# MP-Gadget/MP-Gadget

Measured on AMD Instinct MI355X. Metric: particle-updates/sec (gravity force step: PM + tree build + short-range walk), higher is better.
Workload: dtype f64; 1 GPU; 256^3 DM-only TreePM force step, Nmesh=512, s_zel ICs, all particles active, relative opening criterion (ErrTolForceAcc 0.002), TreeRcut 6, Asmth 1.5; particles=16777216, nmesh=512, parallelism=1 GPU

## Files before the change

mp-gadget_amd/csrc/grav_walk_split.hip:

```cpp
#include "grav_walk.h"
#include <cstdlib>
#include <cstring>
#include <cstdio>
#include <type_traits>

namespace mpg {

namespace {

constexpr int EVAL_BLOCKS = 4;
constexpr int LIST_BLOCKS = 6;

__device__ __forceinline__ double rsqrt_nr(double x)
{
    const double y = __builtin_amdgcn_rsq(x);
    const double e = fma(-(x * y), y, 1.0);
    return fma(y * e, fma(e, 0.375, 0.5), y);
}

template <unsigned long long BITS>
__device__ __forceinline__ double scalar_literal()
{
    unsigned lo, hi;
    asm volatile("s_mov_b32 %0, %2\n\ts_mov_b32 %1, %3" : "=s"(lo), "=s"(hi) : "i"((unsigned)(BITS & 0xffffffffull)), "i"((unsigned)(BITS >> 32)));
    return __hiloint2double((int)hi, (int)lo);
}
#define MPG_K(x) scalar_literal<__builtin_bit_cast(unsigned long long, (double)(x))>()

__device__ __forceinline__ double rcp_nr(double x)
{
    double y = __builtin_amdgcn_rcp(x);
    y = fma(fma(-x, y, 1.0), y, y);
    return fma(fma(-x, y, 1.0), y, y);
}

__device__ __forceinline__ void softened_pair(const double r0, const double r2, const double rinv, const double m, const double h, const double hinv,
                                              const double h3inv, double &fac, double &facpot)
{
    const double r = fma(fma(-r0, r0, r2), 0.5 * rinv, r0);
    const double q = r * hinv;
    const double u = fma(fma(-q, h, r), hinv, q);
    double wpk;
    if(u < 0.5) {
        fac = m * h3inv * (MPG_K(10.666666666667) + u * u * (MPG_K(32.0) * u - MPG_K(38.4)));
        wpk = MPG_K(-2.8) + u * u * (MPG_K(5.333333333333) + u * u * (MPG_K(6.4) * u - MPG_K(9.6)));
    }
    else {
        const double iu = rcp_nr(u);
        fac = m * h3inv * (MPG_K(21.333333333333) - MPG_K(48.0) * u + MPG_K(38.4) * u * u - MPG_K(10.666666666667) * u * u * u -
                           MPG_K(0.066666666667) * (iu * iu * iu));
        wpk = MPG_K(-3.2) + MPG_K(0.066666666667) * iu +
              u * u * (MPG_K(10.666666666667) + u * (MPG_K(-16.0) + u * (MPG_K(9.6) - MPG_K(2.133333333333) * u)));
    }
    facpot = m * hinv * wpk;
}

struct PairTmp {
    double dx, dy, dz, r2, rinv, r, fac, facpot, m;
};

__device__ __forceinline__ void pair_pre(const Src4 s, const double dx, const double dy, const double dz, PairTmp &t)
{
    t.dx = dx;
    t.dy = dy;
    t.dz = dz;
    t.m = s.m;
    t.r2 = dx * dx + dy * dy + dz * dz;
    t.rinv = rsqrt_nr(t.r2);
    t.r = t.r2 * t.rinv;
    const double mr = s.m * t.rinv;
    t.fac = mr * t.rinv * t.rinv;
    t.facpot = -mr;
}

__device__ __forceinline__ void pair_soft(const GravParams &gp, PairTmp &t)
{
    if(t.r2 == 0.0) {
        t.r = 0.0;
        t.fac = t.m * gp.h3inv * 10.666666666667;
        t.facpot = t.m * gp.hinv * -2.8;
    }
    else {
        if(!(t.rinv < 1e150)) {
            t.r = 0.0;
            t.rinv = 0.0;
        }
        softened_pair(t.r, t.r2, t.rinv, t.m, gp.h, gp.hinv, gp.h3inv, t.fac, t.facpot);
    }
}

template <bool POT>
__device__ __forceinline__ void pair_post(const PairTmp &t, const GravParams &gp, const double *__restrict__ wtab, double &ax, double &ay, double &az,
                                          double &pot)
{
    const double ti = t.r * gp.inv_cell_dx;
    const int ix = min((int)ti, NTAB - 1);
    const double w1 = __builtin_amdgcn_fract(ti);
    const double *__restrict__ row = wtab + ix * 2;
    const double2 f = *(const double2 *)row;
    double2 p = f;
    if(POT)
        p = *(const double2 *)(row + 2 * NTAB);
    const double fac = t.fac * fma(w1, f.y, f.x);
    ax = fma(t.dx, fac, ax);
    ay = fma(t.dy, fac, ay);
    az = fma(t.dz, fac, az);
    if(POT)
        pot = fma(t.facpot, fma(w1, p.y, p.x), pot);
}

template <bool POT>
__device__ __forceinline__ void pair_force(const Src4 s, const double dx, const double dy, const double dz, const GravParams &gp,
                                           const double *__restrict__ wtab, double &ax, double &ay,
                                           double &az, double &pot)
{
    PairTmp t;
    pair_pre(s, dx, dy, dz, t);
    if(t.r2 < gp.h2)
        pair_soft(gp, t);
    pair_post<POT>(t, gp, wtab, ax, ay, az, pot);
}

template <bool O32, typename T>
__device__ __forceinline__ T ld(const T *__restrict__ base, const unsigned i)
{
    if(O32)
        return *(const T *)((const char *)base + (size_t)(unsigned)(i * (unsigned)sizeof(T)));
    return base[i];
}

__device__ __forceinline__ void st32(unsigned *__restrict__ base, const unsigned i, const unsigned v)
{
    *(unsigned *)((char *)base + (size_t)(unsigned)(i * 4u)) = v;
}

__device__ __forceinline__ bool any_lane(const bool b) { return __builtin_amdgcn_ballot_w64(b) != 0; }

__device__ __forceinline__ void set_wave_prio(const int p)
{
    if(p == 1)
        __builtin_amdgcn_s_setprio(1);
    else if(p == 2)
        __builtin_amdgcn_s_setprio(2);
    else if(p >= 3)
        __builtin_amdgcn_s_setprio(3);
}

__device__ __forceinline__ double nearest_img(double d, double box, double invbox) { return fma(-rint(d * invbox), box, d); }

struct ChunkIter {
    unsigned lo, hi, first, stride;
    __device__ ChunkIter(unsigned nchunks)
    {
        const unsigned xcd = blockIdx.x & 7;
        const unsigned waves_per_block = blockDim.x >> 6;
        first = (blockIdx.x >> 3) * waves_per_block + (threadIdx.x >> 6);
        stride = (gridDim.x >> 3) * waves_per_block;
        lo = (unsigned)(((uint64_t)nchunks * xcd) >> 3);
        hi = (unsigned)(((uint64_t)nchunks * (xcd + 1)) >> 3);
    }
};

template <int MODE>
__device__ __forceinline__ void node_test_masks(const GravParams &gp, const NodeGeo &g, const Src4 &mom, const bool special,
                                                const bool any_special , const double eff, const double l2, const double inside,
                                                const double ml2, const double px, const double py, const double pz, const double aold,
                                                unsigned long long &m_discard, unsigned long long &m_open, unsigned long long &m_wrap)
{
    double dx, dy, dz, cmax;
    m_wrap = 0ull;
    if(MODE == 0) {
        cmax = fmax(fmax(fabs(nearest_img(g.cx - px, gp.box, gp.invbox)), fabs(nearest_img(g.cy - py, gp.box, gp.invbox))),
                    fabs(nearest_img(g.cz - pz, gp.box, gp.invbox)));
        dx = nearest_img(mom.x - px, gp.box, gp.invbox);
        dy = nearest_img(mom.y - py, gp.box, gp.invbox);
        dz = nearest_img(mom.z - pz, gp.box, gp.invbox);
    }
    else {
        if(MODE == 1) {
            const double kx = rint((g.cx - px) * gp.invbox);
            const double ky = rint((g.cy - py) * gp.invbox);
            const double kz = rint((g.cz - pz) * gp.invbox);
            const double qx = fma(kx, gp.box, px), qy = fma(ky, gp.box, py), qz = fma(kz, gp.box, pz);
            cmax = fmax(fmax(fabs(g.cx - qx), fabs(g.cy - qy)), fabs(g.cz - qz));
            dx = mom.x - qx;
            dy = mom.y - qy;
            dz = mom.z - qz;
            m_wrap = __builtin_amdgcn_ballot_w64(kx != 0.0) | __builtin_amdgcn_ballot_w64(ky != 0.0) | __builtin_amdgcn_ballot_w64(kz != 0.0);
        }
        else {
            cmax = fmax(fmax(fabs(g.cx - px), fabs(g.cy - py)), fabs(g.cz - pz));
            dx = mom.x - px;
            dy = mom.y - py;
            dz = mom.z - pz;
        }
        if(any_special) {
            const double jx = rint((mom.x - px) * gp.invbox), jy = rint((mom.y - py) * gp.invbox), jz = rint((mom.z - pz) * gp.invbox);
            dx = special ? fma(-jx, gp.box, mom.x - px) : dx;
            dy = special ? fma(-jy, gp.box, mom.y - py) : dy;
            dz = special ? fma(-jz, gp.box, mom.z - pz) : dz;
            const unsigned long long m_sp = __builtin_amdgcn_ballot_w64(special);
            m_wrap |= m_sp & (__builtin_amdgcn_ballot_w64(jx != 0.0) | __builtin_amdgcn_ballot_w64(jy != 0.0) | __builtin_amdgcn_ballot_w64(jz != 0.0));
            if(MODE == 2) {
                const double cm = fmax(fmax(fabs(nearest_img(g.cx - px, gp.box, gp.invbox)), fabs(nearest_img(g.cy - py, gp.box, gp.invbox))),
                                       fabs(nearest_img(g.cz - pz, gp.box, gp.invbox)));
                cmax = special ? cm : cmax;
            }
        }
    }
    const double r2 = dx * dx + dy * dy + dz * dz;
    m_discard = __builtin_amdgcn_ballot_w64(r2 > gp.rcut2) & __builtin_amdgcn_ballot_w64(cmax > eff);
    m_open = __builtin_amdgcn_ballot_w64(ml2 > r2 * r2 * aold) | __builtin_amdgcn_ballot_w64(l2 > r2 * gp.bhangle2) | __builtin_amdgcn_ballot_w64(cmax < inside);
}

constexpr int QCAP = 1024;
constexpr int QSLACK = 64 + 7;
constexpr int QSTRIDE_PACKED = 1 + QCAP + QSLACK;

__device__ __forceinline__ unsigned mbcnt64(const unsigned long long b)
{
    return __builtin_amdgcn_mbcnt_hi((unsigned)(b >> 32), __builtin_amdgcn_mbcnt_lo((unsigned)b, 0u));
}

template <int C>
__device__ __forceinline__ void lds_store32(unsigned *p, const unsigned v)
{
    const unsigned a = (unsigned)(size_t)(__attribute__((address_space(3))) unsigned *)p;
    asm volatile("ds_write_b32 %0, %1 offset:%2" : : "v"(a), "v"(v), "n"(4 * C) : "memory");
}

__device__ __forceinline__ int wave_prefix_sum(int x)
{
    x += __builtin_amdgcn_update_dpp(0, x, 0x111, 0xf, 0xf, false);
    x += __builtin_amdgcn_update_dpp(0, x, 0x112, 0xf, 0xf, false);
    x += __builtin_amdgcn_update_dpp(0, x, 0x114, 0xf, 0xf, false);
    x += __builtin_amdgcn_update_dpp(0, x, 0x118, 0xf, 0xf, false);
    x += __builtin_amdgcn_update_dpp(0, x, 0x142, 0xa, 0xf, false);
    x += __builtin_amdgcn_update_dpp(0, x, 0x143, 0xc, 0xf, false);
    return x;
}


struct F32Wave {
    double ox, oy, oz;
    float w1, c1;
    float dr;
    float k4;
    unsigned tweird;
    const float *s_tgtf;
};
constexpr float F32_U = 5.9604644775390625e-8f;

struct WaveTargets {
    int nleaf[8], nnode[8];
    unsigned c_vis[8], c_used[8];
};

template <bool COUNT, int MODE, bool O32, bool PACKQ, bool F32 = false>
__device__ __forceinline__ bool walk_wave8(const TreeView &tv, const GravParams &gp, unsigned *__restrict__ Lw, unsigned *__restrict__ q_node,
                                           unsigned char *__restrict__ q_mask, const double *__restrict__ s_tgt, const int cap, const int lane,
                                           const unsigned live0, WaveTargets &T, unsigned &overflowed, bool &wrapped, unsigned (&c_pp)[8],
                                           const unsigned guard_max, unsigned *__restrict__ ctl, unsigned &st_a, unsigned &st_al,
                                           const F32Wave &W = F32Wave(), unsigned *n_amb = nullptr)
{
    static_assert(!F32 || MODE == 2, "the fp32 pre-classification is written for plain differences");
    unsigned live = live0;
    int sp = 0;
    unsigned guard = 0;
    unsigned long long wmask = 0;
    int maxused = 0;

    auto push_children = [&](const bool pushing, const NodeLinkB &lk, const unsigned openmask) -> bool {
        if(!any_lane(pushing))
            return true;
        const int mine = pushing ? lk.nchild : 0;
        const int upto = wave_prefix_sum(mine);
        const int total = __builtin_amdgcn_readlane(upto, 63);
        if(sp + total > QCAP) {
            overflowed |= live;
            live = 0;
            return false;
        }
        const unsigned at = (unsigned)(sp + upto - mine);
        if constexpr(PACKQ) {
            const unsigned first = (openmask << 24) | (unsigned)lk.firstchild;
            unsigned *qa = q_node + (pushing ? at : (unsigned)(QCAP + lane));
            lds_store32<7>(qa, first + 7u);
            lds_store32<6>(qa, first + 6u);
            lds_store32<5>(qa, first + 5u);
            lds_store32<4>(qa, first + 4u);
            lds_store32<3>(qa, first + 3u);
            lds_store32<2>(qa, first + 2u);
            lds_store32<1>(qa, first + 1u);
            lds_store32<0>(qa, first);
        }
        else if(pushing) {
            const unsigned nm1 = (unsigned)(lk.nchild - 1);
#pragma unroll
            for(unsigned c = 0; c < 8; c++)
                if(c <= nm1) {
                    q_node[at + c] = (unsigned)lk.firstchild + c;
                    q_mask[at + c] = (unsigned char)openmask;
                }
        }
        sp += total;
        return true;
    };

    {
        const int tc = lane & 7, tt = lane >> 3;
        unsigned tmask = live;
        unsigned first = 0u;
        int nch = 1;
        for(int level = 0; tmask != 0u; level++) {
            if(level > 64) {
                if(lane == 0)
                    atomicExch(&ctl[1], 1u);
                return false;
            }
            const bool valid = tc < nch && ((tmask >> tt) & 1u);
            const unsigned my = first + (unsigned)(tc < nch ? tc : 0);
            const NodeGeo g = ld<O32>(tv.geoB, my);
            const Src4 mom = ld<O32>(tv.momB, my);
            const NodeLinkB lk = ld<O32>(tv.linkB, my);
            const double4 tg = *(const double4 *)(s_tgt + 4 * tt);
            const double eff = fma(0.5, g.len, gp.rcut);
            const double l2 = g.len * g.len;
            const bool special = MODE != 0 && valid && level < 2;
            unsigned long long m_discard, m_open, m_wrap;
            node_test_masks<MODE>(gp, g, mom, special, MODE != 0 && level < 2, eff, l2, 0.6 * g.len, mom.m * l2, tg.x, tg.y, tg.z, tg.w, m_discard,
                                  m_open, m_wrap);
            const unsigned long long m_valid = __builtin_amdgcn_ballot_w64(valid);
            const unsigned long long m_leafnode = __builtin_amdgcn_ballot_w64(lk.pcount > 0);
            const unsigned long long m_intnode = ~m_leafnode & __builtin_amdgcn_ballot_w64(lk.nchild > 0);
            const unsigned long long keep = m_valid & ~m_discard;
            const unsigned long long bn = keep & ~m_open, bl = keep & m_open & m_leafnode;
            unsigned long long bpush = keep & m_open & m_intnode;
            if(COUNT) {
                st_a++;
                st_al += (unsigned)nch;
            }
            if(COUNT || (bn | bl) != 0ull) {
                const unsigned ent_val = my;
#pragma unroll
                for(int t = 0; t < 8; t++) {
                    const unsigned long long grp = 0xffull << (8 * t);
                    const unsigned long long bl_t = bl & grp, bn_t = bn & grp;
                    const int kl = __builtin_popcountll(bl_t), kn = __builtin_popcountll(bn_t);
                    if(T.nleaf[t] + T.nnode[t] + kl + kn > cap) {
                        overflowed |= 1u << t;
                        live &= ~(1u << t);
                        bpush &= ~grp;
                        continue;
                    }
                    unsigned *__restrict__ Lt = Lw + (unsigned)(t * cap);
                    if(__builtin_amdgcn_inverse_ballot_w64(bl_t))
                        st32(Lt, __builtin_amdgcn_mbcnt_hi((unsigned)(bl_t >> 32), __builtin_amdgcn_mbcnt_lo((unsigned)bl_t, (unsigned)T.nleaf[t])), ent_val);
                    if(__builtin_amdgcn_inverse_ballot_w64(bn_t))
                        st32(Lt, (unsigned)(cap - 1 - T.nnode[t]) - mbcnt64(bn_t), my);
                    T.nleaf[t] += kl;
                    T.nnode[t] += kn;
                    maxused = max(maxused, T.nleaf[t] + T.nnode[t]);
                    if(COUNT) {
                        T.c_vis[t] += (unsigned)__builtin_popcountll(m_valid & grp);
                        T.c_used[t] += (unsigned)kn;
                        c_pp[t] += __builtin_amdgcn_inverse_ballot_w64(bl_t) ? (unsigned)lk.pcount : 0u;
                    }
                }
            }
            if(MODE != 0)
                wmask |= m_wrap & (bl | bn);
            unsigned om = 0;
#pragma unroll
            for(int t = 0; t < 8; t++)
                om |= (unsigned)((bpush >> (8 * t + tc)) & 1ull) << t;
            const unsigned long long m_opened = __builtin_amdgcn_ballot_w64(lane < 8 && om != 0u);
            if(__builtin_popcountll(m_opened) == 1) {
                const int src = __builtin_ctzll(m_opened);
                tmask = (unsigned)__builtin_amdgcn_readlane((int)om, src);
                first = (unsigned)__builtin_amdgcn_readlane(lk.firstchild, src);
                nch = __builtin_amdgcn_readlane(lk.nchild, src);
            }
            else {
                push_children(lane < 8 && om != 0u, lk, om);
                tmask = 0u;
            }
        }
    }
    while(sp > 0 && live) {
        if(++guard > guard_max) {
            if(lane == 0)
                atomicExch(&ctl[1], 1u);
            return false;
        }
        __builtin_amdgcn_wave_barrier();
        const int n = sp < 64 ? sp : 64;
        unsigned my, mask;
        if constexpr(PACKQ) {
            const unsigned w = q_node[max(sp - 1 - lane, -1)];
            my = w & 0xffffffu;
            mask = w & (live << 24);
        }
        else {
            const bool valid = lane < n;
            const int qi = valid ? sp - 1 - lane : 0;
            my = q_node[qi];
            mask = valid ? (((unsigned)q_mask[qi] & live) << 24) : 0u;
        }
        sp -= n;
        const NodeGeo g = ld<O32>(tv.geoB, my);
        const Src4 mom = ld<O32>(tv.momB, my);
        const NodeLinkB lk = ld<O32>(tv.linkB, my);
        double eff = 0, l2 = 0, inside = 0, ml2 = 0;
        float Cx = 0, Cy = 0, Cz = 0, Sx = 0, Sy = 0, Sz = 0, rE = 0, c2 = 0, c3 = 0, wA = 0, wB = 0, c4 = 0;
        unsigned long long m_nweird = 0ull;
        if constexpr(F32) {
            Cx = (float)(g.cx - W.ox);
            Cy = (float)(g.cy - W.oy);
            Cz = (float)(g.cz - W.oz);
            Sx = (float)(mom.x - W.ox);
            Sy = (float)(mom.y - W.oy);
            Sz = (float)(mom.z - W.oz);
            const float lenf = (float)g.len, mf = (float)mom.m;
            const float l2f = lenf * lenf, ml2f = mf * l2f;
            rE = __builtin_amdgcn_rcpf((12.0f * F32_U) * (lenf + W.dr));
            c2 = -fmaf(0.5f, lenf, (float)gp.rcut) * rE;
            c3 = -(0.6f * lenf) * rE;
            wA = (float)gp.bhangle2 * __builtin_amdgcn_rcpf(lenf * fmaf(64.0f * F32_U, lenf, W.k4));
            const float g4 = wA * l2f * (float)(1.0 / gp.bhangle2);
            wB = __builtin_amdgcn_rsqf(ml2f) * g4;
            c4 = -g4;
            m_nweird = __builtin_amdgcn_ballot_w64(!(ml2f > 1e-30f && ml2f < 1e30f && lenf > 1e-12f && lenf < 1e12f));
        }
        else {
            eff = fma(0.5, g.len, gp.rcut);
            l2 = g.len * g.len;
            inside = 0.6 * g.len;
            ml2 = mom.m * l2;
        }
        const unsigned ent_val = my;
        unsigned openmask = 0;
        if(COUNT) {
            st_a++;
            st_al += (unsigned)n;
        }
        const unsigned long long m_leafnode = __builtin_amdgcn_ballot_w64(lk.pcount > 0);
        const unsigned long long m_intnode = ~m_leafnode & __builtin_amdgcn_ballot_w64(lk.nchild > 0);
        const unsigned long long m_single = __builtin_amdgcn_ballot_w64(lk.pcount == 1);
        auto pass = [&](auto checked_tag) {
            constexpr bool CHECKED = decltype(checked_tag)::value;
            unsigned om = 0u;
#pragma unroll
            for(int t = 7; t >= 0; t--) {
                const unsigned long long m_act = __builtin_amdgcn_ballot_w64((mask & (0x01000000u << t)) != 0u);
                if(m_act == 0ull)
                    continue;
                unsigned ot = 4u * t;
                asm volatile("" : "+v"(ot));
                unsigned long long m_discard, m_open, m_wrap;
                if constexpr(F32) {
                    const float4 tf = *(const float4 *)(W.s_tgtf + ot);
                    const float cdx = Cx - tf.x, cdy = Cy - tf.y, cdz = Cz - tf.z;
                    const float dx = Sx - tf.x, dy = Sy - tf.y, dz = Sz - tf.z;
                    const float cmax = __builtin_fmaxf(__builtin_fmaxf(__builtin_fabsf(cdx), __builtin_fabsf(cdy)), __builtin_fabsf(cdz));
                    const float r2 = fmaf(dz, dz, fmaf(dy, dy, dx * dx));
                    float wT;
                    asm("v_min_f32 %0, %1, %2" : "=v"(wT) : "v"(wA), "v"(wB * tf.w));
                    const float n1 = fmaf(r2, W.w1, W.c1), n2 = fmaf(cmax, rE, c2), n3 = fmaf(cmax, rE, c3), n4 = fmaf(r2, wT, c4);
                    const float dmin = __builtin_fminf(n1, n2), omin = __builtin_fminf(n3, n4);
                    const float amb = __builtin_fminf(__builtin_fabsf(dmin), __builtin_fabsf(omin));
                    m_discard = __builtin_amdgcn_ballot_w64(dmin > 0.0f);
                    m_open = __builtin_amdgcn_ballot_w64(omin < 0.0f);
                    m_wrap = 0ull;
                    const unsigned long long m_amb = (__builtin_amdgcn_ballot_w64(!(amb > 1.0f)) | m_nweird) & m_act;
                    const bool redo = m_amb != 0ull || ((W.tweird >> t) & 1u);
                    if(COUNT || __builtin_expect(redo, 0)) {
                        unsigned my2 = my;
                        asm volatile("" : "+v"(my2));
                        const NodeGeo g2 = ld<O32>(tv.geoB, my2);
                        const Src4 mom2 = ld<O32>(tv.momB, my2);
                        const double4 tg = *(const double4 *)(s_tgt + ot);
                        const double l2d = g2.len * g2.len;
                        unsigned long long e_discard, e_open, e_wrap;
                        node_test_masks<MODE>(gp, g2, mom2, false, false, fma(0.5, g2.len, gp.rcut), l2d, 0.6 * g2.len, mom2.m * l2d, tg.x, tg.y, tg.z,
                                              tg.w, e_discard, e_open, e_wrap);
                        if(COUNT && !redo) {
                            if((((m_discard ^ e_discard) | ((m_open ^ e_open) & ~e_discard)) & m_act) != 0ull && lane == 0)
                                atomicExch(&ctl[1], 3u);
                        }
                        if(COUNT && redo && n_amb)
                            (*n_amb)++;
                        m_discard = e_discard;
                        m_open = e_open;
                    }
                }
                else {
                    const double4 tg = *(const double4 *)(s_tgt + ot);
                    node_test_masks<MODE>(gp, g, mom, false, false, eff, l2, inside, ml2, tg.x, tg.y, tg.z, tg.w, m_discard, m_open, m_wrap);
                }
                const unsigned long long keep = m_act & ~m_discard;
                const unsigned long long bn0 = keep & ~m_open;
                const unsigned long long bl0 = keep & m_open & m_leafnode;
                const unsigned long long bn = bn0 | (bl0 & m_single);
                const unsigned long long bl = bl0 & ~m_single;
                const unsigned long long bpush = keep & m_open & m_intnode;
                const int kl = __builtin_popcountll(bl), kn = __builtin_popcountll(bn);
                if(CHECKED && T.nleaf[t] + T.nnode[t] + kl + kn > cap) {
                    overflowed |= 1u << t;
                    live &= ~(1u << t);
                    continue;
                }
                unsigned *__restrict__ Lt = Lw + (unsigned)(t * cap);
                if(__builtin_amdgcn_inverse_ballot_w64(bl))
                    st32(Lt, __builtin_amdgcn_mbcnt_hi((unsigned)(bl >> 32), __builtin_amdgcn_mbcnt_lo((unsigned)bl, (unsigned)T.nleaf[t])), ent_val);
                if(__builtin_amdgcn_inverse_ballot_w64(bn))
                    st32(Lt, (unsigned)(cap - 1 - T.nnode[t]) - mbcnt64(bn), my);
                T.nleaf[t] += kl;
                T.nnode[t] += kn;
                maxused = max(maxused, T.nleaf[t] + T.nnode[t]);
                om |= __builtin_amdgcn_inverse_ballot_w64(bpush) ? (1u << t) : 0u;
                if(MODE == 1)
                    wmask |= m_wrap & (bl | bn);
                if(COUNT) {
                    T.c_vis[t] += (unsigned)__builtin_popcountll(m_act);
                    T.c_used[t] += (unsigned)__builtin_popcountll(bn0);
                    c_pp[t] += __builtin_amdgcn_inverse_ballot_w64(bl0) ? (unsigned)lk.pcount : 0u;
                }
                __builtin_amdgcn_sched_barrier(0);
            }
            openmask = om;
        };
        if(maxused + 64 > cap)
            pass(std::true_type{});
        else
            pass(std::false_type{});
        if(!push_children(openmask != 0u, lk, openmask))
            break;
    }
    wrapped = wmask != 0ull;
    return true;
}

template <bool COUNT, bool FASTWRAP, bool O32, bool F32, bool PACKQ>
__global__ void __launch_bounds__(256, LIST_BLOCKS) k_walk_lists8(const TreeView tv, const GravParams gp, const WalkIO io, unsigned *__restrict__ lists,
                                                      int2 *__restrict__ counts, const int cap, const int64_t slot0, const int64_t nslots,
                                                      unsigned *__restrict__ ctl, int *__restrict__ ovf)
{
    constexpr int QSTRIDE = PACKQ ? QSTRIDE_PACKED : QCAP;
    __shared__ unsigned s_qnode[4 * QSTRIDE];
    __shared__ __attribute__((aligned(32))) double s_tgt4[4 * 8 * 4];
    __shared__ __attribute__((aligned(16))) float s_tgtf4[F32 ? 4 * 8 * 4 : 4];
    set_wave_prio(io.list_prio);
    const int lane = threadIdx.x & 63;
    unsigned *q_node = s_qnode + (threadIdx.x >> 6) * QSTRIDE;
    unsigned char *q_mask = nullptr;
    if constexpr(PACKQ) {
        if(lane == 0)
            q_node[0] = 0u;
        q_node++;
    }
    else {
        __shared__ unsigned char s_qmask[4 * QCAP];
        q_mask = s_qmask + (threadIdx.x >> 6) * QCAP;
    }
    double *s_tgt = s_tgt4 + (threadIdx.x >> 6) * 32;
    const unsigned nchunks = (unsigned)((nslots + 7) / 8);
    const ChunkIter it(nchunks);
    const unsigned guard_max = (unsigned)min((long long)(8ll * (tv.nnodes + 1024)), 0x7fffffffll);
    const double face = gp.rcut + 0.002 * gp.box;
    unsigned long long n_pp = 0, n_vis = 0, n_used = 0, n_le = 0, n_se = 0;
    unsigned st_a = 0, st_al = 0, n_amb = 0, n_f32w = 0;
    float *s_tgtf = s_tgtf4 + (F32 ? (threadIdx.x >> 6) * 32 : 0);

    for(unsigned chunk = it.lo + it.first; chunk < it.hi; chunk += it.stride) {
        const int64_t rel = (int64_t)chunk * 8 + (lane & 7);
        const bool tvalid = lane < 8 && rel < nslots;
        int ci = -1;
        double vx = 0, vy = 0, vz = 0, vaold = 0;
        if(tvalid) {
            const int64_t slot = slot0 + rel;
            ci = io.targets ? io.targets[slot] : tv.order[slot];
            vx = io.pos[3 * (int64_t)ci + 0];
            vy = io.pos[3 * (int64_t)ci + 1];
            vz = io.pos[3 * (int64_t)ci + 2];
            double old = 0;
            if(io.oldacc)
                old = io.oldacc[ci];
            else if(io.prev_accel) {
                double s2 = 0;
                for(int j = 0; j < 3; j++) {
                    const double a = io.prev_accel[3 * (int64_t)ci + j] + (io.gravpm ? io.gravpm[3 * (int64_t)ci + j] : 0.0);
                    s2 += a * a;
                }
                old = sqrt(s2) / gp.G;
            }
            vaold = gp.use_bh ? __builtin_inf() : gp.errtol * old;
        }
        const bool near_face = tvalid && (fmin(fmin(vx, vy), vz) < face || fmax(fmax(vx, vy), vz) > gp.box - face);
        const unsigned live0 = (unsigned)(__builtin_amdgcn_ballot_w64(tvalid) & 0xffull);
        WaveTargets T;
        unsigned c_pp[8];
        __builtin_amdgcn_wave_barrier();
        if(lane < 8)
            *(double4 *)(s_tgt + 4 * lane) = make_double4(vx, vy, vz, vaold);
        __builtin_amdgcn_wave_barrier();
#pragma unroll
        for(int t = 0; t < 8; t++) {
            T.nleaf[t] = T.nnode[t] = 0;
            T.c_vis[t] = T.c_used[t] = 0u;
            c_pp[t] = 0u;
        }
        unsigned *__restrict__ L = lists + (size_t)__builtin_amdgcn_readfirstlane((int)chunk) * (size_t)cap * 8;
        unsigned overflowed = 0;
        bool wrapped = false;
        bool ok;
        if(FASTWRAP) {
            if(!any_lane(near_face)) {
                if constexpr(F32) {
                    F32Wave W;
                    const int l0 = live0 ? __builtin_ctz(live0) : 0;
                    W.ox = __shfl(vx, l0);
                    W.oy = __shfl(vy, l0);
                    W.oz = __shfl(vz, l0);
                    double dmax = tvalid ? fmax(fmax(fabs(vx - W.ox), fabs(vy - W.oy)), fabs(vz - W.oz)) : 0.0;
                    for(int off = 1; off < 8; off <<= 1)
                        dmax = fmax(dmax, __shfl_xor(dmax, off));
                    const double D = __shfl(dmax, 0) * 1.000001;
                    const double E1 = 24.0 * (double)F32_U * gp.rcut2 + 20.0 * (double)F32_U * D * gp.rcut;
                    W.w1 = (float)(1.0 / E1);
                    W.c1 = -(float)gp.rcut2 * W.w1;
                    W.dr = (float)((D + gp.rcut) * 1.000001);
                    W.k4 = (float)(32.0 * (double)F32_U * D * sqrt(gp.bhangle2) * 1.000001);
                    const bool tw = tvalid && !(vaold == 0.0 || vaold == __builtin_inf() || (vaold > 1e-30 && vaold < 1e30));
                    W.tweird = (unsigned)(__builtin_amdgcn_ballot_w64(tw) & 0xffull);
                    W.s_tgtf = s_tgtf;
                    __builtin_amdgcn_wave_barrier();
                    if(lane < 8)
                        *(float4 *)(s_tgtf + 4 * lane) = make_float4((float)(vx - W.ox), (float)(vy - W.oy), (float)(vz - W.oz), (float)sqrt(vaold));
                    __builtin_amdgcn_wave_barrier();
                    n_f32w++;
                    ok = walk_wave8<COUNT, 2, O32, PACKQ, true>(tv, gp, L, q_node, q_mask, s_tgt, cap, lane, live0, T, overflowed, wrapped, c_pp, guard_max, ctl, st_a,
                                                         st_al, W, &n_amb);
                }
                else
                    ok = walk_wave8<COUNT, 2, O32, PACKQ>(tv, gp, L, q_node, q_mask, s_tgt, cap, lane, live0, T, overflowed, wrapped, c_pp, guard_max, ctl, st_a, st_al);
            }
            else
                ok = walk_wave8<COUNT, 1, O32, PACKQ>(tv, gp, L, q_node, q_mask, s_tgt, cap, lane, live0, T, overflowed, wrapped, c_pp, guard_max, ctl, st_a, st_al);
        }
        else
            ok = walk_wave8<COUNT, 0, O32, PACKQ>(tv, gp, L, q_node, q_mask, s_tgt, cap, lane, live0, T, overflowed, wrapped, c_pp, guard_max, ctl, st_a, st_al);
        if(!ok)
            return;
        int nl = 0, nn = 0;
#pragma unroll
        for(int t = 0; t < 8; t++)
            if(lane == t) {
                nl = T.nleaf[t];
                nn = T.nnode[t];
            }
        if(tvalid) {
            const bool overflow = (overflowed >> lane) & 1u;
            if(io.cost)
                io.cost[ci] = (float)(8 * (overflow ? cap : nl) + nn + 3 * (nl + nn));
            if(overflow) {
                counts[rel] = make_int2(-1, 0);
                ovf[atomicAdd(&ctl[0], 1u)] = ci;
            }
            else {
                counts[rel] = make_int2(nl | (wrapped ? (1 << 30) : 0), nn);
                if((unsigned)(nl + nn) > ctl[2])
                    atomicMax(&ctl[2], (unsigned)(nl + nn));
            }
        }
        if(COUNT) {
#pragma unroll
            for(int t = 0; t < 8; t++)
                if(!((overflowed >> t) & 1u)) {
                    n_pp += c_pp[t];
                    if(lane == 0) {
                        n_vis += T.c_vis[t];
                        n_used += T.c_used[t];
                        n_le += (unsigned)T.nleaf[t];
                        n_se += (unsigned)T.nnode[t];
                    }
                }
        }
    }
    if(COUNT) {
        unsigned long long c0 = n_pp, c1 = n_vis, c2 = n_used, c3 = lane == 0 ? st_a : 0u, c4 = lane == 0 ? st_al : 0u;
        for(int off = 32; off > 0; off >>= 1) {
            c0 += __shfl_down(c0, off);
            c1 += __shfl_down(c1, off);
            c2 += __shfl_down(c2, off);
            c3 += __shfl_down(c3, off);
            c4 += __shfl_down(c4, off);
        }
        if(lane == 0) {
            atomicAdd(&io.counters[5], n_le);
            atomicAdd(&io.counters[6], n_se);
            atomicAdd(&io.counters[0], c0);
            atomicAdd(&io.counters[1], c1);
            atomicAdd(&io.counters[2], c2);
            atomicAdd(&io.counters[3], c3);
            atomicAdd(&io.counters[4], c4);
            if(F32 && n_amb)
                atomicAdd(&io.counters[12], (unsigned long long)n_amb);
            if(F32 && n_f32w)
                atomicAdd(&io.counters[13], (unsigned long long)n_f32w);
        }
    }
}

constexpr int RING_STRIDE = 17;

template <bool POT, bool WRAP, bool O32>
__device__ __forceinline__ void eval_lists(const TreeView &tv, const GravParams &gp, const unsigned *__restrict__ L, const int cap, const int nleaf,
                                           const int nnode, const int s, const int gshift, const double px,
                                           const double py, const double pz, const double *__restrict__ s_wtab, unsigned *__restrict__ ring_g,
                                           double &ax, double &ay, double &az, double &pot)
{
    const unsigned empty = (unsigned)tv.nnodes;
    const unsigned s32 = (unsigned)s * 32u;
#define MPG_LOAD(EJ, SV)                                                                        \
    {                                                                                           \
        const unsigned ej_ = (EJ);                                                              \
        if(O32)                                                                                 \
            SV = *(const Src4 *)((const char *)tv.srcL + (size_t)((ej_ << 8) + s32));           \
        else                                                                                    \
            SV = tv.srcL[(size_t)ej_ * 8 + (size_t)s];                                          \
    }
#define MPG_EVAL(SV)                                                              \
    {                                                                             \
        __builtin_amdgcn_sched_barrier(0);                                        \
        double dx_ = SV.x - px, dy_ = SV.y - py, dz_ = SV.z - pz;                 \
        if(WRAP) {                                                                \
            dx_ = nearest_img(dx_, gp.box, gp.invbox);                            \
            dy_ = nearest_img(dy_, gp.box, gp.invbox);                            \
            dz_ = nearest_img(dz_, gp.box, gp.invbox);                            \
        }                                                                         \
        pair_force<POT>(SV, dx_, dy_, dz_, gp, s_wtab, ax, ay, az, pot);           \
        asm volatile("" : "+v"(ax), "+v"(ay), "+v"(az), "+v"(pot));               \
        __builtin_amdgcn_sched_barrier(0);                                        \
    }
    {
        const unsigned ls = (unsigned)((gshift >> 3) * cap + s);
#define MPG_LEAF_AT(E0) (ls + (unsigned)(E0))
        __builtin_amdgcn_wave_barrier();
        ring_g[s] = (s < nleaf) ? ld<true>(L, MPG_LEAF_AT(0)) : empty;
        unsigned ent_n = (8 + s < nleaf) ? ld<true>(L, MPG_LEAF_AT(8)) : empty;
        __builtin_amdgcn_wave_barrier();
        unsigned eb = ring_g[1];
        Src4 A, B;
        MPG_LOAD(ring_g[0], A);
        int wmax = nleaf;
        for(int off = 8; off < 64; off <<= 1)
            wmax = max(wmax, __shfl_xor(wmax, off));
        wmax = __builtin_amdgcn_readfirstlane(wmax);
        Src4 Cq = A;
        MPG_LOAD(eb, B);
        int staged = 1;
#pragma unroll 1
        for(int e = 0; e < wmax; e += 3) {
            if(e + 4 >= 8 * staged) {
                ring_g[(staged & 1) * 8 + s] = ent_n;
                ent_n = ((staged + 1) * 8 + s < nleaf) ? ld<true>(L, MPG_LEAF_AT((staged + 1) * 8)) : empty;
                staged++;
                __builtin_amdgcn_wave_barrier();
            }
            const unsigned e2 = ring_g[(e + 2) & 15], e3 = ring_g[(e + 3) & 15], e4 = ring_g[(e + 4) & 15];
            MPG_LOAD(e2, Cq);
            MPG_EVAL(A);
            MPG_LOAD(e3, A);
            MPG_EVAL(B);
            MPG_LOAD(e4, B);
            MPG_EVAL(Cq);
        }
    }
    if(any_lane(nnode > 0)) {
        const unsigned NONE = (unsigned)tv.nnodes;
        const unsigned top = (unsigned)((gshift >> 3) * cap + cap - 1 - s);
#define MPG_NODE_AT(R0) (top - (unsigned)(R0))
#define MPG_NODE_ENT(R0) (((R0) + s < nnode) ? ld<true>(L, MPG_NODE_AT(R0)) : NONE)
        Src4 Sa = ld<O32>(tv.momB, MPG_NODE_ENT(0));
        Src4 Sb = ld<O32>(tv.momB, MPG_NODE_ENT(8));
        Src4 Sc;
        unsigned nx = MPG_NODE_ENT(16), ny = MPG_NODE_ENT(24), nz = MPG_NODE_ENT(32);
#pragma unroll 1
        for(int r0 = 0;; r0 += 24) {
            if(!any_lane(r0 < nnode))
                break;
            Sc = ld<O32>(tv.momB, nx);
            nx = MPG_NODE_ENT(r0 + 40);
            MPG_EVAL(Sa);
            if(!any_lane(r0 + 8 < nnode))
                break;
            Sa = ld<O32>(tv.momB, ny);
            ny = MPG_NODE_ENT(r0 + 48);
            MPG_EVAL(Sb);
            if(!any_lane(r0 + 16 < nnode))
                break;
            Sb = ld<O32>(tv.momB, nz);
            nz = MPG_NODE_ENT(r0 + 56);
            MPG_EVAL(Sc);
        }
#undef MPG_NODE_ENT
    }
#undef MPG_LOAD
#undef MPG_EVAL
#undef MPG_LEAF_AT
#undef MPG_NODE_AT
}

__device__ __attribute__((noinline)) double potential_postprocess(double pot, const double m, const double h, const double cbrtrho0, const double G)
{
    pot += m / (h / 2.8);
    pot -= 2.8372975 * pow(m, 2.0 / 3) * cbrtrho0;
    return pot * G;
}

template <bool POT, bool FASTWRAP, bool O32>
__global__ void __launch_bounds__(256, EVAL_BLOCKS) k_walk_eval(const TreeView tv, const GravParams gp, const WalkIO io, const unsigned *__restrict__ lists,
                                                    const int2 *__restrict__ counts, const int cap, const int64_t slot0, const int64_t nslots)
{
    constexpr int ROW = POT ? 4 : 2;
    __shared__ __attribute__((aligned(16))) double s_wtab[NTAB * ROW];
    __shared__ unsigned s_ring[4 * 8 * RING_STRIDE];
    set_wave_prio(io.eval_prio);
    for(int i = threadIdx.x; i < NTAB; i += blockDim.x) {
        const bool last = i == NTAB - 1;
        s_wtab[i * 2 + 0] = last ? 0.0 : (double)io.tab_force[i];
        s_wtab[i * 2 + 1] = last ? 0.0 : (double)io.tab_force[i + 1] - (double)io.tab_force[i];
        if(POT) {
            s_wtab[2 * NTAB + i * 2 + 0] = last ? 0.0 : (double)io.tab_pot[i];
            s_wtab[2 * NTAB + i * 2 + 1] = last ? 0.0 : (double)io.tab_pot[i + 1] - (double)io.tab_pot[i];
        }
    }
    __syncthreads();

    const int lane = threadIdx.x & 63;
    const int grp = lane >> 3, s = lane & 7;
    const int gshift = grp * 8;
    unsigned *__restrict__ ring_g = s_ring + ((threadIdx.x >> 6) * 8 + grp) * RING_STRIDE;
    const unsigned nchunks = (unsigned)((nslots + 7) / 8);
    const ChunkIter it(nchunks);

    for(unsigned chunk = it.lo + it.first; chunk < it.hi; chunk += it.stride) {
        const int64_t rel = (int64_t)chunk * 8 + grp;
        bool valid = rel < nslots;
        const int64_t slot = slot0 + rel;
        int ci = -1;
        double px = 0, py = 0, pz = 0;
        int nleaf = 0, nnode = 0;
        bool wrapped = false;
        if(valid) {
            const int2 c = counts[rel];
            if(c.x < 0)
                valid = false;
            else {
                nleaf = c.x & 0x3fffffff;
                wrapped = (c.x >> 30) & 1;
                nnode = c.y;
                ci = io.targets ? io.targets[slot] : tv.order[slot];
                px = io.pos[3 * (int64_t)ci + 0];
                py = io.pos[3 * (int64_t)ci + 1];
                pz = io.pos[3 * (int64_t)ci + 2];
            }
        }
        const unsigned *__restrict__ L = lists + (size_t)__builtin_amdgcn_readfirstlane((int)chunk) * (size_t)cap * 8;
        double ax = 0, ay = 0, az = 0, pot = 0;
        if(!FASTWRAP || any_lane(wrapped))
            eval_lists<POT, true, O32>(tv, gp, L, cap, nleaf, nnode, s, gshift, px, py, pz, s_wtab, ring_g, ax, ay, az, pot);
        else
            eval_lists<POT, false, O32>(tv, gp, L, cap, nleaf, nnode, s, gshift, px, py, pz, s_wtab, ring_g, ax, ay, az, pot);
        for(int off = 1; off < 8; off <<= 1) {
            ax += __shfl_xor(ax, off);
            ay += __shfl_xor(ay, off);
            az += __shfl_xor(az, off);
            if(POT)
                pot += __shfl_xor(pot, off);
        }
        if(valid && s == 0) {
            io.accel[3 * (int64_t)ci + 0] = ax * gp.G;
            io.accel[3 * (int64_t)ci + 1] = ay * gp.G;
            io.accel[3 * (int64_t)ci + 2] = az * gp.G;
            if(POT && io.potential)
                io.potential[ci] = potential_postprocess(pot, (double)io.mass[ci], gp.h, gp.cbrtrho0, gp.G);
        }
    }
}

int grid_blocks(WalkScratch &ws, const void *kern, int64_t nchunks, int chunks_per_wave)
{
    if(ws.num_cu == 0) {
        int dev = 0;
        MPG_HIP(hipGetDevice(&dev));
        MPG_HIP(hipDeviceGetAttribute(&ws.num_cu, hipDeviceAttributeMultiprocessorCount, dev));
    }
    const int64_t need = (nchunks + 3) / 4;
    int64_t nblocks;
    if(chunks_per_wave > 0)
        nblocks = (need + chunks_per_wave - 1) / chunks_per_wave;
    else {
        int occ = 0;
        MPG_HIP(hipOccupancyMaxActiveBlocksPerMultiprocessor(&occ, kern, 256, 0));
        if(occ < 1)
            occ = 1;
        if(occ > 8)
            occ = 8;
        nblocks = (int64_t)ws.num_cu * occ;
        if(nblocks > need)
            nblocks = need;
    }
    return (int)((nblocks + 7) / 8 * 8);
}

template <bool POT, bool COUNT, bool FASTWRAP, bool O32>
void launch_split_t(const TreeView &tv, const GravParams &gp, const WalkIO &io, WalkScratch &ws, hipStream_t st)
{
    const char *f32_e = getenv("MPG_LISTS_F32");
    const bool f32_env = f32_e && f32_e[0] == '1';
    const bool f32 = FASTWRAP && f32_env && gp.bhangle2 > 1e-6 && gp.bhangle2 < 1e6 && gp.rcut > 1e-12 && gp.rcut < 1e12 && gp.box < 1e12;
    const char *pq_e = getenv("MPG_LISTS_PACKQ");
    const bool packq = tv.nnodes + 1 <= (1ll << 24) && !(pq_e && pq_e[0] == '0');
    auto kl = (FASTWRAP && f32) ? (packq ? k_walk_lists8<COUNT, FASTWRAP, O32, FASTWRAP, true> : k_walk_lists8<COUNT, FASTWRAP, O32, FASTWRAP, false>)
                                : (packq ? k_walk_lists8<COUNT, FASTWRAP, O32, false, true> : k_walk_lists8<COUNT, FASTWRAP, O32, false, false>);
    auto ke = k_walk_eval<POT, FASTWRAP, O32>;
    if(const char *e = getenv("MPG_LIST_CAP"))
        ws.split_cap = atoi(e) / 8 * 8;
    const int cap = ws.split_cap;
    static const size_t long_bytes = getenv("MPG_SPLIT_BYTES_LONG") ? (size_t)atoll(getenv("MPG_SPLIT_BYTES_LONG")) : ((size_t)16 << 30);
    const size_t area = cap >= 4096 ? (ws.split_bytes < long_bytes ? ws.split_bytes : long_bytes) : ws.split_bytes;
    int64_t slice = (int64_t)(area / ((size_t)cap * sizeof(unsigned))) / 2048 * 2048;
    if(slice < 65536)
        slice = 65536;
    if(slice > ws.split_slice)
        slice = ws.split_slice;
    if(const char *e = getenv("MPG_SPLIT_SLICE"))
        slice = atoll(e);
    const int64_t nmax = io.ntargets < slice ? io.ntargets : slice;
    const int64_t nslices = (io.ntargets + slice - 1) / slice;
    static const int ov_env = getenv("MPG_SPLIT_OVERLAP") ? (getenv("MPG_SPLIT_OVERLAP")[0] == '0' ? 0 : 1) : -1;
    const bool overlap = (ov_env >= 0 ? ov_env != 0 : ws.split_overlap) && nslices > 1;
    const size_t lists_sz = (size_t)((nmax + 15) / 16) * 16 * (size_t)cap, counts_sz = (size_t)nmax + 8;
    ws.split_lists.reserve(lists_sz * (overlap ? 2 : 1));
    ws.split_counts.reserve(counts_sz * (overlap ? 2 : 1));
    ws.split_ovf.reserve((size_t)io.ntargets);
    if(overlap && !ws.split_stream) {
        MPG_HIP(hipStreamCreateWithFlags(&ws.split_stream, hipStreamNonBlocking));
        for(int k = 0; k < 2; k++) {
            MPG_HIP(hipEventCreateWithFlags(&ws.ev_lists[k], hipEventDisableTiming));
            MPG_HIP(hipEventCreateWithFlags(&ws.ev_eval[k], hipEventDisableTiming));
        }
        MPG_HIP(hipEventCreateWithFlags(&ws.ev_begin, hipEventDisableTiming));
    }
    static const int cpw_env = getenv("MPG_SPLIT_CPW") ? atoi(getenv("MPG_SPLIT_CPW")) : -1;
    const int cpw = cpw_env >= 0 ? cpw_env : ws.split_chunks_per_wave;
    hipStream_t sl = overlap ? ws.split_stream : st;
    if(overlap) {
        MPG_HIP(hipEventRecord(ws.ev_begin, st));
        MPG_HIP(hipStreamWaitEvent(sl, ws.ev_begin, 0));
    }
    int64_t i = 0;
    for(int64_t s0 = 0; s0 < io.ntargets; s0 += slice, i++) {
        const int64_t ns = (io.ntargets - s0 < slice) ? io.ntargets - s0 : slice;
        const int64_t nchunks = (ns + 7) / 8;
        const int b = overlap ? (int)(i & 1) : 0;
        unsigned *lists = ws.split_lists.p + (size_t)b * lists_sz;
        int2 *counts = ws.split_counts.p + (size_t)b * counts_sz;
        if(overlap && i >= 2)
            MPG_HIP(hipStreamWaitEvent(sl, ws.ev_eval[b], 0));
        static const bool split_time = getenv("MPG_SPLIT_TIME") != nullptr;
        hipEvent_t te[3] = {nullptr, nullptr, nullptr};
        if(split_time) {
            for(auto &e : te)
                MPG_HIP(hipEventCreate(&e));
            MPG_HIP(hipEventRecord(te[0], sl));
        }
        hipLaunchKernelGGL(kl, dim3((unsigned)grid_blocks(ws, (const void *)kl, nchunks, (COUNT && cpw > 0 && cpw < 8) ? 8 : cpw)), dim3(256), 0, sl, tv, gp, io,
                           lists, counts, cap, s0, ns, ws.ctr.p, ws.split_ovf.p);
        if(split_time)
            MPG_HIP(hipEventRecord(te[1], sl));
        if(overlap) {
            MPG_HIP(hipEventRecord(ws.ev_lists[b], sl));
            MPG_HIP(hipStreamWaitEvent(st, ws.ev_lists[b], 0));
        }
        if(ws.ev_mid && nslices == 1 && !overlap) {
            MPG_HIP(hipEventRecord(ws.ev_mid, st));
            ws.mid_recorded = true;
        }
        if(ws.ev_before_eval && i == 0)
            MPG_HIP(hipStreamWaitEvent(st, ws.ev_before_eval, 0));
        hipLaunchKernelGGL(ke, dim3((unsigned)grid_blocks(ws, (const void *)ke, nchunks, cpw)), dim3(256), 0, st, tv, gp, io, lists, counts, cap, s0,
                           ns);
        if(overlap)
            MPG_HIP(hipEventRecord(ws.ev_eval[b], st));
        if(split_time) {
            MPG_HIP(hipEventRecord(te[2], st));
            MPG_HIP(hipEventSynchronize(te[2]));
            float ml = 0, me = 0;
            MPG_HIP(hipEventElapsedTime(&ml, te[0], te[1]));
            MPG_HIP(hipEventElapsedTime(&me, te[1], te[2]));
            fprintf(stderr, "SPLIT_TIME targets %lld lists %.3f ms eval %.3f ms\n", (long long)ns, ml, me);
            for(auto &e : te)
                MPG_HIP(hipEventDestroy(e));
        }
    }
    MPG_HIP(hipGetLastError());
}

}

void launch_grav_walk_split(const TreeView &tv, const GravParams &gp, const WalkIO &io, bool want_pot, bool count, bool fastwrap, WalkScratch &ws,
                            hipStream_t st)
{
    if(io.ntargets == 0)
        return;
    MPG_CHECK(tv.npart < (1ll << 29), "split walk: more than 2^29 particles in one tree");
    ws.ctr.reserve(16);
    MPG_CHECK(tv.srcL != nullptr, "split walk: the tree carries no padded leaf sources (TreeBuilder::ensure_leaf_pad)");
    const bool o32 = !ws.split_offsets64 && (tv.npart + tv.nnodes + 64) * 32 < (1ll << 32) && (tv.nnodes + 2) * 256 < (1ll << 32);
#define MPG_WS(P, C)                                                \
    do {                                                            \
        if(fastwrap) {                                              \
            if(o32)                                                 \
                launch_split_t<P, C, true, true>(tv, gp, io, ws, st);  \
            else                                                    \
                launch_split_t<P, C, true, false>(tv, gp, io, ws, st); \
        }                                                           \
        else                                                        \
            launch_split_t<P, C, false, false>(tv, gp, io, ws, st); \
    } while(0)
    unsigned ctl[4] = {0, 0, 0, 0};
    for(;;) {
        MPG_HIP(hipMemsetAsync(ws.ctr.p, 0, 16 * sizeof(unsigned), st));
        if(want_pot) {
            if(count)
                MPG_WS(true, true);
            else
                MPG_WS(true, false);
        }
        else {
            if(count)
                MPG_WS(false, true);
            else
                MPG_WS(false, false);
        }
        MPG_HIP(hipMemcpyAsync(ctl, ws.ctr.p, sizeof(ctl), hipMemcpyDeviceToHost, st));
        MPG_HIP(hipStreamSynchronize(st));
        MPG_CHECK(ctl[1] == 0, "short-range walk (list construction) aborted by its loop guard (corrupt tree?)");
        if(!count && (int64_t)ctl[0] * 5 > io.ntargets && ws.split_cap < 8192) {
            ws.split_cap = ws.split_cap * 4 < 8192 ? ws.split_cap * 4 : 8192;
            ws.mid_recorded = false;
            ws.ev_mid = nullptr;
            continue;
        }
        break;
    }
#undef MPG_WS
    ws.split_last_overflow = ctl[0];
    ws.split_last_maxlen = ctl[2];
    if(ctl[0] > 0) {
        WalkIO io2 = io;
        io2.targets = ws.split_ovf.p;
        io2.ntargets = ctl[0];
        launch_grav_walk_coop(tv, gp, io2, want_pot, count, fastwrap, ws, st);
        MPG_CHECK(walk_coop_error(ws, st) == 0, "short-range walk (fallback for long lists) aborted by its loop guard");
        if((int64_t)ctl[0] * 50 > io.ntargets && ws.split_cap < 8192) {
            ws.split_cap *= 2;
            if((int64_t)ctl[0] * 5 > io.ntargets && ws.split_cap < 8192)
                ws.split_cap *= 2;
        }
    }
}

}
```

Baseline: 255.2 million particles/s.

## Cut walk register pressure: drop checked/unchecked pass split, raise list occupancy, split potential postprocess

The list-building walk no longer tracks maxused or instantiates separate checked and unchecked passes; the capacity check now always runs. Target loads switch to explicit LDS vector loads from opaque base addresses, and the common list-kernel variant gets a higher launch-bounds occupancy target. Potential postprocessing moves out of the eval kernel into a separate small kernel. The aim is lower VGPR pressure and more waves in flight, at the cost of an extra per-lane compare and an extra kernel launch when potentials are requested.

```diff
diff --git a/mp-gadget_amd/csrc/grav_walk_split.hip b/mp-gadget_amd/csrc/grav_walk_split.hip
--- a/mp-gadget_amd/csrc/grav_walk_split.hip
+++ b/mp-gadget_amd/csrc/grav_walk_split.hip
@@ -222,6 +222,19 @@
     return __builtin_amdgcn_mbcnt_hi((unsigned)(b >> 32), __builtin_amdgcn_mbcnt_lo((unsigned)b, 0u));
 }
 
+typedef double lds_d4 __attribute__((ext_vector_type(4)));
+typedef float lds_f4 __attribute__((ext_vector_type(4)));
+__device__ __forceinline__ double4 lds_load_double4(const unsigned a)
+{
+    const lds_d4 v = *(const __attribute__((address_space(3))) lds_d4 *)(size_t)a;
+    return make_double4(v.x, v.y, v.z, v.w);
+}
+__device__ __forceinline__ float4 lds_load_float4(const unsigned a)
+{
+    const lds_f4 v = *(const __attribute__((address_space(3))) lds_f4 *)(size_t)a;
+    return make_float4(v.x, v.y, v.z, v.w);
+}
+
 template <int C>
 __device__ __forceinline__ void lds_store32(unsigned *p, const unsigned v)
 {
@@ -268,7 +281,6 @@
     int sp = 0;
     unsigned guard = 0;
     unsigned long long wmask = 0;
-    int maxused = 0;
 
     auto push_children = [&](const bool pushing, const NodeLinkB &lk, const unsigned openmask) -> bool {
         if(!any_lane(pushing))
@@ -360,7 +372,6 @@
                         st32(Lt, (unsigned)(cap - 1 - T.nnode[t]) - mbcnt64(bn_t), my);
                     T.nleaf[t] += kl;
                     T.nnode[t] += kn;
-                    maxused = max(maxused, T.nleaf[t] + T.nnode[t]);
                     if(COUNT) {
                         T.c_vis[t] += (unsigned)__builtin_popcountll(m_valid & grp);
                         T.c_used[t] += (unsigned)kn;
@@ -440,6 +451,13 @@
         }
         const unsigned ent_val = my;
         unsigned openmask = 0;
+        unsigned tgt_lds = (unsigned)(size_t)(const __attribute__((address_space(3))) double *)s_tgt;
+        asm volatile("" : "+v"(tgt_lds));
+        [[maybe_unused]] unsigned tgtf_lds = 0u;
+        if constexpr(F32) {
+            tgtf_lds = (unsigned)(size_t)(const __attribute__((address_space(3))) float *)W.s_tgtf;
+            asm volatile("" : "+v"(tgtf_lds));
+        }
         if(COUNT) {
             st_a++;
             st_al += (unsigned)n;
@@ -447,19 +465,17 @@
         const unsigned long long m_leafnode = __builtin_amdgcn_ballot_w64(lk.pcount > 0);
         const unsigned long long m_intnode = ~m_leafnode & __builtin_amdgcn_ballot_w64(lk.nchild > 0);
         const unsigned long long m_single = __builtin_amdgcn_ballot_w64(lk.pcount == 1);
-        auto pass = [&](auto checked_tag) {
-            constexpr bool CHECKED = decltype(checked_tag)::value;
+        auto pass = [&]() {
             unsigned om = 0u;
 #pragma unroll
             for(int t = 7; t >= 0; t--) {
                 const unsigned long long m_act = __builtin_amdgcn_ballot_w64((mask & (0x01000000u << t)) != 0u);
                 if(m_act == 0ull)
                     continue;
-                unsigned ot = 4u * t;
-                asm volatile("" : "+v"(ot));
+#define MPG_TGT() lds_load_double4(tgt_lds + 32u * (unsigned)t)
                 unsigned long long m_discard, m_open, m_wrap;
                 if constexpr(F32) {
-                    const float4 tf = *(const float4 *)(W.s_tgtf + ot);
+                    const float4 tf = lds_load_float4(tgtf_lds + 16u * (unsigned)t);
                     const float cdx = Cx - tf.x, cdy = Cy - tf.y, cdz = Cz - tf.z;
                     const float dx = Sx - tf.x, dy = Sy - tf.y, dz = Sz - tf.z;
                     const float cmax = __builtin_fmaxf(__builtin_fmaxf(__builtin_fabsf(cdx), __builtin_fabsf(cdy)), __builtin_fabsf(cdz));
@@ -479,7 +495,7 @@
                         asm volatile("" : "+v"(my2));
                         const NodeGeo g2 = ld<O32>(tv.geoB, my2);
                         const Src4 mom2 = ld<O32>(tv.momB, my2);
-                        const double4 tg = *(const double4 *)(s_tgt + ot);
+                        const double4 tg = MPG_TGT();
                         const double l2d = g2.len * g2.len;
                         unsigned long long e_discard, e_open, e_wrap;
                         node_test_masks<MODE>(gp, g2, mom2, false, false, fma(0.5, g2.len, gp.rcut), l2d, 0.6 * g2.len, mom2.m * l2d, tg.x, tg.y, tg.z,
@@ -495,7 +511,7 @@
                     }
                 }
                 else {
-                    const double4 tg = *(const double4 *)(s_tgt + ot);
+                    const double4 tg = MPG_TGT();
                     node_test_masks<MODE>(gp, g, mom, false, false, eff, l2, inside, ml2, tg.x, tg.y, tg.z, tg.w, m_discard, m_open, m_wrap);
                 }
                 const unsigned long long keep = m_act & ~m_discard;
@@ -505,7 +521,7 @@
                 const unsigned long long bl = bl0 & ~m_single;
                 const unsigned long long bpush = keep & m_open & m_intnode;
                 const int kl = __builtin_popcountll(bl), kn = __builtin_popcountll(bn);
-                if(CHECKED && T.nleaf[t] + T.nnode[t] + kl + kn > cap) {
+                if((T.nleaf[t] + kl) + (T.nnode[t] + kn) > cap) {
                     overflowed |= 1u << t;
                     live &= ~(1u << t);
                     continue;
@@ -517,7 +533,6 @@
                     st32(Lt, (unsigned)(cap - 1 - T.nnode[t]) - mbcnt64(bn), my);
                 T.nleaf[t] += kl;
                 T.nnode[t] += kn;
-                maxused = max(maxused, T.nleaf[t] + T.nnode[t]);
                 om |= __builtin_amdgcn_inverse_ballot_w64(bpush) ? (1u << t) : 0u;
                 if(MODE == 1)
                     wmask |= m_wrap & (bl | bn);
@@ -528,12 +543,10 @@
                 }
                 __builtin_amdgcn_sched_barrier(0);
             }
+#undef MPG_TGT
             openmask = om;
         };
-        if(maxused + 64 > cap)
-            pass(std::true_type{});
-        else
-            pass(std::false_type{});
+        pass();
         if(!push_children(openmask != 0u, lk, openmask))
             break;
     }
@@ -542,7 +555,7 @@
 }
 
 template <bool COUNT, bool FASTWRAP, bool O32, bool F32, bool PACKQ>
-__global__ void __launch_bounds__(256, LIST_BLOCKS) k_walk_lists8(const TreeView tv, const GravParams gp, const WalkIO io, unsigned *__restrict__ lists,
+__global__ void __launch_bounds__(256, (!COUNT && !FASTWRAP && PACKQ) ? LIST_BLOCKS + 1 : LIST_BLOCKS) k_walk_lists8(const TreeView tv, const GravParams gp, const WalkIO io, unsigned *__restrict__ lists,
                                                       int2 *__restrict__ counts, const int cap, const int64_t slot0, const int64_t nslots,
                                                       unsigned *__restrict__ ctl, int *__restrict__ ovf)
 {
@@ -885,9 +898,20 @@
             io.accel[3 * (int64_t)ci + 1] = ay * gp.G;
             io.accel[3 * (int64_t)ci + 2] = az * gp.G;
             if(POT && io.potential)
-                io.potential[ci] = potential_postprocess(pot, (double)io.mass[ci], gp.h, gp.cbrtrho0, gp.G);
-        }
-    }
+                io.potential[ci] = pot;
+        }
+    }
+}
+
+__global__ void __launch_bounds__(256) k_walk_potpost(const TreeView tv, const GravParams gp, const WalkIO io, const int2 *__restrict__ counts,
+                                                      const int64_t slot0, const int64_t nslots)
+{
+    const int64_t rel = (int64_t)blockIdx.x * blockDim.x + threadIdx.x;
+    if(rel >= nslots || counts[rel].x < 0)
+        return;
+    const int64_t slot = slot0 + rel;
+    const int ci = io.targets ? io.targets[slot] : tv.order[slot];
+    io.potential[ci] = potential_postprocess(io.potential[ci], (double)io.mass[ci], gp.h, gp.cbrtrho0, gp.G);
 }
 
 int grid_blocks(WalkScratch &ws, const void *kern, int64_t nchunks, int chunks_per_wave)
@@ -993,6 +1017,8 @@
             MPG_HIP(hipStreamWaitEvent(st, ws.ev_before_eval, 0));
         hipLaunchKernelGGL(ke, dim3((unsigned)grid_blocks(ws, (const void *)ke, nchunks, cpw)), dim3(256), 0, st, tv, gp, io, lists, counts, cap, s0,
                            ns);
+        if(POT && io.potential)
+            hipLaunchKernelGGL(k_walk_potpost, dim3((unsigned)((ns + 255) / 256)), dim3(256), 0, st, tv, gp, io, counts, s0, ns);
         if(overlap)
             MPG_HIP(hipEventRecord(ws.ev_eval[b], st));
         if(split_time) {
```

Result: no change. 256.1 million particles/s (median of 6 runs) (+0.3%).
